# ZYM-PKU/UDiffText

Measured on AMD Instinct MI355X. Metric: 512x512 50-step denoised images/sec (UDiffText hot path: conditioner + 50 CFG Euler steps + VAE decode), higher is better.
Workload: dtype bf16; 1 GPU; 512x512, 50 Euler/DDIM(eta 0) steps, CFG 5.0, 9-char labels, noise_iters 0; global batch 4 per step sharded over 1 GPU(s) = 4 images per GPU in micro-batches of 4: every UNet call runs ONE batch of 4 (8 samples with CFG); 3 such batch(es) in flight per GPU on separate launch streams; BASELINE.json configs[1]; global_batch=4, weights=synthetic (name-keyed recipe), 1361.2 M parameters, launch=hipGraph replay of the sampler steps, in_flight=3, batches_per_unet_call=1

## Files before the change

### include/udt_kernels.h

```cpp
#ifndef UDT_KERNELS_H
#define UDT_KERNELS_H

#include <stddef.h>
#include <stdint.h>

#ifdef __cplusplus
extern "C" {
#endif

typedef enum {
  UDT_OK = 0,
  UDT_ERR_BAD_SHAPE = -1,
  UDT_ERR_BAD_ARG = -2,
  UDT_ERR_WORKSPACE = -3,
  UDT_ERR_HIP = -4,
  UDT_ERR_NO_DEVICE = -5,
  UDT_ERR_ASYNC = -6
} udt_status;

typedef enum {
  UDT_DTYPE_F32 = 0,
  UDT_DTYPE_BF16 = 1,
  UDT_DTYPE_FP8_E4M3 = 2
} udt_dtype;
// ... 94 lines not shown
                          int32_t batch, int32_t nq, int32_t nk,
                          int32_t ldq, int32_t ldk, int32_t ldv, int32_t ldo,
                          int64_t q_bstride, int64_t k_bstride, int64_t v_bstride, int64_t o_bstride,
                          float scale, void* workspace, size_t workspace_bytes, void* stream);

int udt_mattn_fwd(const void* q, const void* k, const void* v, void* o, const float* mask, const uint8_t* kpm,
                  int32_t batch, int32_t heads, int32_t head_dim, int32_t nq, int32_t lk,
                  int32_t ldq, int32_t ldk, int32_t ldv, int32_t ldo, int32_t ldmask,
                  int64_t q_bstride, int64_t k_bstride, int64_t v_bstride, int64_t o_bstride, float scale, void* stream);

int32_t udt_tattn_hp(int32_t heads);
int udt_tattn_prepare(const void* kv, int32_t ldkv, const void* wq, int32_t ldwq, const void* wo, int32_t ldwo,
                      const float* gamma, const float* beta, void* A, float* sc, void* BmT, int32_t B, int32_t L,
                      int32_t C, int32_t heads, float scale, void* stream);
int udt_tattn_fused(const void* x, void* out, const void* A, const float* sc, const void* BmT, const float* bias,
                    int32_t B, int32_t n_tok, int32_t C, int32_t heads, int32_t zero_samples, float eps, void* stream);
int32_t udt_tattn_rowstat_parts(int32_t B, int32_t n_tok, int32_t C);
int udt_tattn_fused_q8(const void* x, void* out, const void* A, const float* sc, const void* BmT, const float* bias,
                       int32_t B, int32_t n_tok, int32_t C, int32_t heads, int32_t zero_samples, float eps, void* q8_out,
                       void* q8_scale, float* rowstat_out, void* stream);

int udt_softmax_rows(void* x, int64_t rows, int32_t cols, int32_t ld, void* stream);

int32_t udt_gn_nchunks(int64_t HW, int32_t C);
int udt_gn_stats(const void* x, const void* x2, float* partials, int32_t B, int64_t HW, int32_t C, int32_t C2,
                 int32_t G, void* stream);
int udt_gn_apply(const void* x, const void* x2, void* y, const float* partials, const float* gamma,
                 const float* beta, int32_t B, int64_t HW, int32_t C, int32_t C2, int32_t G, float eps, int32_t act,
                 void* stream);
int32_t udt_gn_strip_ok(int32_t B, int64_t HW, int32_t C1, int32_t C2, int32_t G);
int udt_gn_strip(const void* x, const void* x2, void* y, const float* gamma, const float* beta, int32_t B, int64_t HW,
// ... 175 lines not shown
```

### udifftext_amd/csrc/common.h

```cpp
#pragma once
#include <hip/hip_runtime.h>
#include <stdint.h>
#include "../../include/udt_kernels.h"

typedef __attribute__((ext_vector_type(8))) __bf16 bf16x8_t;
typedef __attribute__((ext_vector_type(2))) __bf16 bf16x2_t;
typedef __attribute__((ext_vector_type(2))) float f32x2;
typedef __attribute__((ext_vector_type(4))) float f32x4;
typedef __attribute__((ext_vector_type(16))) float f32x16;
typedef __attribute__((ext_vector_type(2))) uint32_t u32x2;
typedef __attribute__((ext_vector_type(4))) uint32_t u32x4;

#define UDT_DEVINL __device__ __forceinline__

#ifdef UDT_MEASURE
#define UDT_DBG(flags, bit) ((((flags) >> (bit)) & 1) != 0)
#else
#define UDT_DBG(flags, bit) false
#endif

UDT_DEVINL float bf16_bits_to_f32(uint32_t v) { return __uint_as_float(v << 16); }
UDT_DEVINL float bf16_lo(uint32_t packed) { return __uint_as_float(packed << 16); }
UDT_DEVINL float bf16_hi(uint32_t packed) { return __uint_as_float(packed & 0xffff0000u); }

// ... 162 lines not shown
UDT_DEVINL float xor32_sum(float v) {
  const auto r = __builtin_amdgcn_permlane32_swap(__builtin_bit_cast(unsigned, v), __builtin_bit_cast(unsigned, v), false, false);
  return __builtin_bit_cast(float, (unsigned)r[0]) + __builtin_bit_cast(float, (unsigned)r[1]);
}

int udt_set_hip_error(hipError_t e);
const uint16_t* udt_zero_page();

struct UdtProfScope {
  int cls; hipStream_t s; void* rec;
  UdtProfScope(int cls_, hipStream_t s_);
  ~UdtProfScope();
};

void udt_prof_tag(void* rec, const char* tag);

#define UDT_CHECK_LAUNCH()                                   \
  do {                                                       \
    hipError_t _e = hipGetLastError();                       \
    if (_e != hipSuccess) return udt_set_hip_error(_e);      \
  } while (0)
```

### udifftext_amd/csrc/gemm.hip

```cpp
#include "common.h"
#include <stdio.h>
#include <stdlib.h>
#include <string.h>
#include <atomic>
#include <cmath>

hipError_t udt_lean_launch_gemm(int cfg, const void* lparams, int smem, int G, int geglu, int ln, hipStream_t s);
hipError_t udt_lean_launch_conv3(const void* c3params, hipStream_t s);

namespace {
#include "tile_common.h"

struct GemmParams {
  const uint16_t* a;
  const uint16_t* a2;
  const uint16_t* w;
  const uint16_t* zero;
  const float* bias;
  const uint16_t* res;
  const float* rowvec;
  void* out;
  const float* colscale;
  const float* in_scsh;
  float* colstats;
// ... 966 lines not shown
  if (lean_plan(d, lt, true)) {
    rows = lt.stats_rows;
    slots = lt.tiles_m * (lt.bm / lt.stats_rows);
    return true;
  }
  return false;
}
}

extern "C" int udt_debug_set(const char* key, int32_t value) {
  if (!key) return UDT_ERR_BAD_ARG;
  if (!strcmp(key, "n_block")) { g_n_block.store(value); return UDT_OK; }
  if (!strcmp(key, "rows_epi")) { g_rows_epi.store(value ? 1 : 0); return UDT_OK; }
  if (!strcmp(key, "lean")) { g_lean.store(value < 0 ? -2 : value); return UDT_OK; }
  if (!strcmp(key, "rowres")) { g_rowres.store(value < 0 ? 1 : (value ? 1 : 0)); return UDT_OK; }
  if (!strcmp(key, "wide_lanes_eff")) { g_wide_lanes_eff.store(value < 0 ? -2 : value); return UDT_OK; }
  if (!strcmp(key, "conv_n4")) { g_conv_n4.store(value < 0 ? -2 : (value ? 1 : 0)); return UDT_OK; }
  if (!strcmp(key, "lean256_lanes")) { g_lean256_lanes.store(value < 0 ? -2 : (value ? 1 : 0)); return UDT_OK; }
  if (!strcmp(key, "lean_splitk")) { g_lean_splitk.store(value); return UDT_OK; }
  if (!strcmp(key, "share_splitk")) { g_share_splitk.store(value < 0 ? -2 : (value ? 1 : 0)); return UDT_OK; }
  if (!strcmp(key, "lean_conv")) { g_lean_conv.store(value < 0 ? -1 : (value ? 1 : 0)); return UDT_OK; }
  if (!strcmp(key, "wide_conv")) { g_wide_conv.store(value < 0 ? -1 : (value ? 1 : 0)); return UDT_OK; }
#ifdef UDT_MEASURE
  if (!strcmp(key, "lconv_dbg")) { g_lconv_dbg.store(value); return UDT_OK; }
  static const struct { const char* k; int bit; } bits[] = {{"no_xchg", 28}, {"no_epi", 27}, {"no_store", 26}, {"no_res", 25},
                                                            {"no_bias", 24}, {"no_fast", 22}};
  for (const auto& b : bits)
    if (!strcmp(key, b.k)) {
      int cur = g_dbg_bits.load();
      g_dbg_bits.store((cur & ~(1 << b.bit)) | (value ? (1 << b.bit) : 0));
// ... 390 lines not shown
```

### udifftext_amd/csrc/tattn.hip

```cpp
#include "common.h"
#include <stdio.h>
#include <stdlib.h>

namespace {

constexpr int TA_THREADS = 512;
constexpr int TA_WAVES = TA_THREADS / 64;

struct TattnParams {
  const uint16_t* x;
  uint16_t* out;
  const uint16_t* A;
  const float* sc;
  const uint16_t* BmT;
  const float* bias;
  const uint16_t* zero;
  int M, C, hp, n_tok, zero_samples;
  int nsplit;
  float eps;
  uint8_t* q8_out;
  uint32_t* q8_scale;
  float* rowstat_out;
};

UDT_DEVINL f32x16 zero16() {
  f32x16 z;
#pragma unroll
  for (int r = 0; r < 16; ++r) z[r] = 0.f;
  return z;
}

template <int TT, int NKT, int NKS, bool Q8 = false>
__global__ void __launch_bounds__(TA_THREADS) tattn_fused_kernel(const TattnParams p) {
  extern __shared__ __attribute__((aligned(16))) char smem[];
  constexpr int C = NKT * 64, hp = NKS * 16;
  constexpr int nkt = NKT;
  constexpr int TA_AHEAD = NKT <= 10 ? NKT : 8;
  char* const xs = smem;
  float* const stats = reinterpret_cast<float*>(smem + (size_t)nkt * TT * 128);
  const int prs = hp * 2 + 16;
  char* const pl = reinterpret_cast<char*>(stats + TT * 2);
  const int tid = threadIdx.x;
  const int wave = __builtin_amdgcn_readfirstlane(tid >> 6);
  const int lane = tid & 63;
  const int l31 = lane & 31, hi = lane >> 5;
  const long long tok0 = (long long)blockIdx.x * TT;
  const int b = (int)(tok0 / p.n_tok);
  const uint16_t* xg = p.x + tok0 * C;
  uint16_t* og = p.out + tok0 * C;
  float* const rst = reinterpret_cast<float*>(pl + (size_t)TT * prs);
  const int ct_lo = (int)blockIdx.y * (C >> 5) / p.nsplit, ct_hi = ((int)blockIdx.y + 1) * (C >> 5) / p.nsplit;
  auto q8_row_stats = [&]() {
    __syncthreads();
    if (tid < TT && tok0 + tid < p.M) {
      float s = 0.f, q = 0.f;
      for (int ct = ct_lo; ct < ct_hi; ++ct) {
        const f32x2 v = *reinterpret_cast<const f32x2*>(rst + ((size_t)tid * (C >> 5) + ct) * 2);
        s += v[0];
        q += v[1];
      }
      f32x2 o = {s, q};
      reinterpret_cast<f32x2*>(p.rowstat_out)[(long long)blockIdx.y * p.M + tok0 + tid] = o;
    }
  };


  const uint16_t* Ab = p.A + (long long)b * hp * C;
  constexpr int jt = hp >> 5;
  constexpr int tiles1 = jt * (TT / 32);
// ... 2 lines not shown
  if (live && wave < tiles1) {
    const uint16_t* arow = Ab + (long long)(wave / (TT / 32)) * (32 * C) + lane * 8;
#pragma unroll
    for (int u = 0; u < TA_AHEAD; ++u)
#pragma unroll
      for (int ks = 0; ks < 4; ++ks) ar[u][ks] = *reinterpret_cast<const bf16x8_t*>(arow + (u * 4 + ks) * 512);
  }

  {
    const int pieces = nkt * (TT / 8);
    const int l3 = lane >> 3, ps = lane & 7;
    for (int pc = wave; pc < pieces; pc += TA_WAVES) {
      const int kt = pc / (TT / 8), rg = pc - kt * (TT / 8);
      const int row = rg * 8 + l3;
      const int slot = ps ^ ((row >> 1) & 7);
      const uint16_t* src = (tok0 + row < p.M) ? (xg + (long long)row * C + kt * 64 + slot * 8) : p.zero;
      glds16(src, xs + (size_t)pc * 1024);
    }
    wait_vmcnt0();
  }
  __syncthreads();

  if (b < p.zero_samples) {
    const int ch_lo = ct_lo * 4, ch_hi = ct_hi * 4;
    const int nch = ch_hi - ch_lo;
    for (int i0 = 0; i0 < TT * nch; i0 += TA_THREADS) {
      const int i = i0 + tid;
      const bool act = i < TT * nch;
      const int row = act ? i / nch : 0, ch = ch_lo + (act ? i - row * nch : 0);
      const bool ok = act && tok0 + row < p.M;
      const int kt = ch >> 3, s = ch & 7;
      const u32x4 v = *reinterpret_cast<const u32x4*>(xs + ((size_t)kt * TT + row) * 128 + ((s ^ ((row >> 1) & 7)) << 4));
      const f32x4 b0 = *reinterpret_cast<const f32x4*>(p.bias + ch * 8), b1 = *reinterpret_cast<const f32x4*>(p.bias + ch * 8 + 4);
      const float f[8] = {bf16_lo(v[0]) + b0[0], bf16_hi(v[0]) + b0[1], bf16_lo(v[1]) + b0[2], bf16_hi(v[1]) + b0[3],
                          bf16_lo(v[2]) + b1[0], bf16_hi(v[2]) + b1[1], bf16_lo(v[3]) + b1[2], bf16_hi(v[3]) + b1[3]};
      u32x4 o = {pack_bf16x2(f[0], f[1]), pack_bf16x2(f[2], f[3]), pack_bf16x2(f[4], f[5]), pack_bf16x2(f[6], f[7])};
      if (ok) *reinterpret_cast<u32x4*>(og + (long long)row * C + ch * 8) = o;
      if constexpr (Q8) {
        uint32_t sb;
        const u32x2 q8 = mx8_quant_row8(f, sb);
        float ps = 0.f, pq = 0.f;
#pragma unroll
        for (int j = 0; j < 8; ++j) ps += f[j], pq += f[j] * f[j];
        ps = dpp_add<0xB1>(ps); pq = dpp_add<0xB1>(pq);
        ps = dpp_add<0x4E>(ps); pq = dpp_add<0x4E>(pq);
// ... 61 lines not shown
      bf16x8_t af[4], xf[4];
#pragma unroll
      for (int ks = 0; ks < 4; ++ks) {
        af[ks] = ar[u][ks];
        xf[ks] = lds_read_frag(xrow + (((ks * 2 + hi) ^ swz) << 4));
      }
      if (kt + TA_AHEAD < nkt) {
#pragma unroll
        for (int ks = 0; ks < 4; ++ks) ar[u][ks] = *reinterpret_cast<const bf16x8_t*>(arow + ((kt + TA_AHEAD) * 4 + ks) * 512);
      }
#pragma unroll
      for (int ks = 0; ks < 4; ++ks) acc = mfma32(af[ks], xf[ks], acc);
    }
    const float mean = stats[row * 2], rstd = stats[row * 2 + 1];
    float sv[16];
#pragma unroll
    for (int r4 = 0; r4 < 4; ++r4) {
      const int j = ct * 32 + 8 * r4 + 4 * hi;
      const f32x4 c0 = *reinterpret_cast<const f32x4*>(scb + j * 2), c1 = *reinterpret_cast<const f32x4*>(scb + j * 2 + 4);
      sv[r4 * 4 + 0] = rstd * (acc[r4 * 4 + 0] - mean * c0[0]) + c0[1];
      sv[r4 * 4 + 1] = rstd * (acc[r4 * 4 + 1] - mean * c0[2]) + c0[3];
      sv[r4 * 4 + 2] = rstd * (acc[r4 * 4 + 2] - mean * c1[0]) + c1[1];
      sv[r4 * 4 + 3] = rstd * (acc[r4 * 4 + 3] - mean * c1[2]) + c1[3];
    }
#pragma unroll
    for (int h2 = 0; h2 < 2; ++h2) {
      float mx = sv[h2 * 8];
#pragma unroll
      for (int r = 1; r < 8; ++r) mx = fmaxf(mx, sv[h2 * 8 + r]);
      mx = fmaxf(mx, __shfl_xor(mx, 32));
      float sum = 0.f;
#pragma unroll
      for (int r = 0; r < 8; ++r) {
        sv[h2 * 8 + r] = __expf(sv[h2 * 8 + r] - mx);
        sum += sv[h2 * 8 + r];
      }
      sum += __shfl_xor(sum, 32);
      const float inv = 1.0f / sum;
#pragma unroll
      for (int r = 0; r < 8; ++r) sv[h2 * 8 + r] *= inv;
    }
#pragma unroll
    for (int r4 = 0; r4 < 4; ++r4) {
      const int j = ct * 32 + 8 * r4 + 4 * hi;
      u32x2 pk = {pack_bf16x2(sv[r4 * 4], sv[r4 * 4 + 1]), pack_bf16x2(sv[r4 * 4 + 2], sv[r4 * 4 + 3])};
      *reinterpret_cast<u32x2*>(pl + (size_t)row * prs + j * 2) = pk;
    }
  }
  __syncthreads();

  const uint16_t* Bb = p.BmT + (long long)b * C * hp;
  const int tiles2 = (ct_hi - ct_lo) * (TT / 32);
  constexpr int nks = NKS;
  for (int t = wave; t < tiles2; t += TA_WAVES) {
    const int rt = t % (TT / 32), ct = ct_lo + t / (TT / 32);
    const int row = rt * 32 + l31;
    const uint16_t* brow = Bb + (long long)ct * (32 * hp) + lane * 8;
    const char* prow = pl + (size_t)row * prs + hi * 16;
    f32x16 acc = zero16();
    bf16x8_t bn[NKS];
#pragma unroll
    for (int i = 0; i < NKS; ++i) bn[i] = *reinterpret_cast<const bf16x8_t*>(brow + i * 512);
#pragma unroll
    for (int ks = 0; ks < nks; ++ks) {
      const bf16x8_t pf = *reinterpret_cast<const bf16x8_t*>(prow + ks * 32);
      acc = mfma32(bn[ks], pf, acc);
    }
    {
      const bool rok = tok0 + row < p.M;
      const int swz = (row >> 1) & 7;
      float v[16];
#pragma unroll
      for (int r4 = 0; r4 < 4; ++r4) {
        const int c = ct * 32 + 8 * r4 + 4 * hi;
        const f32x4 bv = *reinterpret_cast<const f32x4*>(p.bias + c);
        const int kt = c >> 6, sl = (c & 63) >> 3;
        const u32x2 xr = *reinterpret_cast<const u32x2*>(xs + ((size_t)kt * TT + row) * 128 + ((sl ^ swz) << 4) + (c & 7) * 2);
        v[r4 * 4 + 0] = acc[r4 * 4 + 0] + bv[0] + bf16_lo(xr[0]);
        v[r4 * 4 + 1] = acc[r4 * 4 + 1] + bv[1] + bf16_hi(xr[0]);
        v[r4 * 4 + 2] = acc[r4 * 4 + 2] + bv[2] + bf16_lo(xr[1]);
        v[r4 * 4 + 3] = acc[r4 * 4 + 3] + bv[3] + bf16_hi(xr[1]);
        u32x2 pk = {pack_bf16x2(v[r4 * 4 + 0], v[r4 * 4 + 1]), pack_bf16x2(v[r4 * 4 + 2], v[r4 * 4 + 3])};
        if (rok) *reinterpret_cast<u32x2*>(og + (long long)row * C + c) = pk;
      }
// ... 7 lines not shown
        pq = xor32_sum(pq);
        if (rok) {
          const long long m = tok0 + row;
#pragma unroll
          for (int r4 = 0; r4 < 4; ++r4) *reinterpret_cast<uint32_t*>(p.q8_out + m * C + ct * 32 + 8 * r4 + 4 * hi) = q[r4];
          if (hi == 0) {
            reinterpret_cast<uint8_t*>(p.q8_scale)[((long long)(ct >> 2) * p.M + m) * 4 + (ct & 3)] = (uint8_t)sb;
            f32x2 st2 = {ps, pq};
            *reinterpret_cast<f32x2*>(rst + ((size_t)row * (C >> 5) + ct) * 2) = st2;
          }
        }
      }
    }
  }
  if constexpr (Q8) q8_row_stats();
}

__global__ void __launch_bounds__(256) tattn_prepare_a_kernel(const uint16_t* __restrict__ kv, int ldkv, const uint16_t* __restrict__ wq,
                                                              int ldwq, const float* __restrict__ gamma, const float* __restrict__ beta,
                                                              uint16_t* __restrict__ A, float* __restrict__ sc, int L, int C, int hp,
                                                              int heads, float scale) {
  __shared__ float kvec[64];
  __shared__ float red[2][4];
  const int j = blockIdx.x, b = blockIdx.y, t = threadIdx.x;
  const int h = j >> 4, i = j & 15;
  uint16_t* const Ab = A + (long long)b * hp * C;
  const int nkt = C >> 6;
  auto aoff = [&](int k) {
    return ((((long long)(j >> 5) * nkt + (k >> 6)) * 4 + ((k >> 4) & 3)) * 64 + ((k >> 3) & 1) * 32 + (j & 31)) * 8 + (k & 7);
  };
// ... 58 lines not shown
  hipStream_t s = reinterpret_cast<hipStream_t>(stream);
  UdtProfScope prof(3, s);
  hipLaunchKernelGGL(tattn_prepare_a_kernel, dim3(hp, B), dim3(256), 0, s, reinterpret_cast<const uint16_t*>(kv), ldkv,
                     reinterpret_cast<const uint16_t*>(wq), ldwq, gamma, beta, reinterpret_cast<uint16_t*>(A), sc, L, C, hp, heads, scale);
  UDT_CHECK_LAUNCH();
  const long long n = (long long)B * C * hp;
  hipLaunchKernelGGL(tattn_prepare_b_kernel, dim3((unsigned)((n + 255) / 256)), dim3(256), 0, s,
                     reinterpret_cast<const uint16_t*>(kv), ldkv, C, reinterpret_cast<const uint16_t*>(wo), ldwo,
                     reinterpret_cast<uint16_t*>(BmT), B, L, C, hp, heads);
  UDT_CHECK_LAUNCH();
  return UDT_OK;
}

namespace {
int tattn_tt(int C) { return C >= 640 ? 32 : 64; }
int tattn_nsplit(int M, int TT) {
  const unsigned grid = (unsigned)(M / TT);
  constexpr unsigned target = 256u;
  int nsplit = 1;
  while (nsplit < 8 && grid * nsplit < target) nsplit *= 2;
  return nsplit;
}

int tattn_launch(const void* x, void* out, const void* A, const float* sc, const void* BmT, const float* bias, int32_t B, int32_t n_tok,
                 int32_t C, int32_t heads, int32_t zero_samples, float eps, void* q8_out, void* q8_scale, float* rowstat_out, void* stream) {
  if (!x || !out || !bias || (zero_samples < B && (!A || !sc || !BmT))) return UDT_ERR_BAD_ARG;
  if (B <= 0 || n_tok <= 0 || heads <= 0 || C != heads * 64 || C > 1280 || zero_samples < 0 || zero_samples > B) return UDT_ERR_BAD_SHAPE;
  const int TT = tattn_tt(C);
  if (n_tok % TT != 0) return UDT_ERR_BAD_SHAPE;
  const bool q8 = q8_out != nullptr;
  if (q8 && (!q8_scale || !rowstat_out || C % 128 != 0)) return UDT_ERR_BAD_ARG;
  TattnParams p;
  p.x = reinterpret_cast<const uint16_t*>(x); p.out = reinterpret_cast<uint16_t*>(out);
  p.A = reinterpret_cast<const uint16_t*>(A); p.sc = sc; p.BmT = reinterpret_cast<const uint16_t*>(BmT); p.bias = bias;
  p.zero = udt_zero_page();
  if (!p.zero) return UDT_ERR_HIP;
  p.M = B * n_tok; p.C = C; p.hp = udt_tattn_hp(heads); p.n_tok = n_tok; p.zero_samples = zero_samples; p.eps = eps;
  p.q8_out = reinterpret_cast<uint8_t*>(q8_out); p.q8_scale = reinterpret_cast<uint32_t*>(q8_scale); p.rowstat_out = rowstat_out;
  const size_t smem = (size_t)TT * C * 2 + (size_t)TT * 2 * sizeof(float) + (size_t)TT * (p.hp * 2 + 16) + (q8 ? (size_t)TT * (C / 32) * 8 : 0);
  hipStream_t s = reinterpret_cast<hipStream_t>(stream);
  UdtProfScope prof(3, s);
  if (prof.rec) {
    char tag[96];
    snprintf(tag, sizeof(tag), "tattn_fused%s B=%d n=%d C=%d zero=%d", q8 ? "+q8" : "", B, n_tok, C, zero_samples);
    udt_prof_tag(prof.rec, tag);
  }
  static bool attr_done[5] = {false, false, false, false, false};
  const unsigned grid = (unsigned)(p.M / TT);
  p.nsplit = tattn_nsplit(p.M, TT);
  const void* fn = nullptr;
  int which = -1;
  if (C == 320 && p.hp == 96 && !q8) { fn = reinterpret_cast<const void*>(tattn_fused_kernel<64, 5, 6>); which = 0; }
  else if (C == 640 && p.hp == 160) { fn = q8 ? reinterpret_cast<const void*>(tattn_fused_kernel<32, 10, 10, true>) : reinterpret_cast<const void*>(tattn_fused_kernel<32, 10, 10>); which = q8 ? 3 : 1; }
  else if (C == 1280 && p.hp == 320) { fn = q8 ? reinterpret_cast<const void*>(tattn_fused_kernel<32, 20, 20, true>) : reinterpret_cast<const void*>(tattn_fused_kernel<32, 20, 20>); which = q8 ? 4 : 2; }
  else return UDT_ERR_BAD_SHAPE;
  if (!attr_done[which]) {
    hipError_t e = hipFuncSetAttribute(fn, hipFuncAttributeMaxDynamicSharedMemorySize, 128 * 1024);
    if (e != hipSuccess) return udt_set_hip_error(e);
    attr_done[which] = true;
  }
  void* args[] = {&p};
  hipError_t el = hipLaunchKernel(fn, dim3(grid, p.nsplit), dim3(TA_THREADS), args, smem, s);
  if (el != hipSuccess) return udt_set_hip_error(el);
  UDT_CHECK_LAUNCH();
  return UDT_OK;
}
}

extern "C" int udt_tattn_fused(const void* x, void* out, const void* A, const float* sc, const void* BmT, const float* bias,
                               int32_t B, int32_t n_tok, int32_t C, int32_t heads, int32_t zero_samples, float eps, void* stream) {
  return tattn_launch(x, out, A, sc, BmT, bias, B, n_tok, C, heads, zero_samples, eps, nullptr, nullptr, nullptr, stream);
}

extern "C" int32_t udt_tattn_rowstat_parts(int32_t B, int32_t n_tok, int32_t C) {
  if (B <= 0 || n_tok <= 0 || (C != 640 && C != 1280)) return 0;
  const int TT = tattn_tt(C);
  if (n_tok % TT != 0) return 0;
  return tattn_nsplit(B * n_tok, TT);
}

extern "C" int udt_tattn_fused_q8(const void* x, void* out, const void* A, const float* sc, const void* BmT, const float* bias,
                                  int32_t B, int32_t n_tok, int32_t C, int32_t heads, int32_t zero_samples, float eps, void* q8_out,
                                  void* q8_scale, float* rowstat_out, void* stream) {
  if (!q8_out) return UDT_ERR_BAD_ARG;
  return tattn_launch(x, out, A, sc, BmT, bias, B, n_tok, C, heads, zero_samples, eps, q8_out, q8_scale, rowstat_out, stream);
}
```

### udifftext_amd/lib.py

```python
from __future__ import annotations

import ctypes as C
import os

_HERE = os.path.dirname(os.path.abspath(__file__))
LIB_PATH = os.path.join(_HERE, "libudt_kernels.so")

GEMM_OUT_F32 = 1 << 0
DTYPE_F32, DTYPE_BF16, DTYPE_FP8_E4M3 = 0, 1, 2
GEMM_GEGLU = 1 << 1
GEMM_RELU = 1 << 2
GEMM_TRANSPOSED = 1 << 3
GEMM_CONV = 1 << 4
GEMM_SILU_OUT = 1 << 5
GEMM_MX8 = 1 << 7

PROF_CONV3X3, PROF_GEMM, PROF_ATTN, PROF_XATTN, PROF_NORM, PROF_ELEMENTWISE = range(6)


class GemmDesc(C.Structure):
    _fields_ = [
        ("a", C.c_void_p), ("a2", C.c_void_p), ("w", C.c_void_p), ("bias", C.c_void_p),
        ("residual", C.c_void_p), ("rowvec", C.c_void_p), ("out", C.c_void_p),
        ("M", C.c_int32), ("N", C.c_int32), ("K", C.c_int32),
# ... 63 lines not shown
    "udt_attn_rowv_fwd": (C.c_int, [_vp, _vp, _vp, _vp, _i32, _i32, _i32, _i32, _i32, _i32, _i32, _i32,
                                    _i64, _i64, _i64, _i64, _f32, _vp]),
    "udt_attn_rowv_q8_fwd": (C.c_int, [_vp, _vp, _vp, _vp, _i32, _i32, _i32, _i32, _i32, _i32, _i32, _i32,
                                       _i64, _i64, _i64, _i64, _f32, _vp, _vp, _i32, _vp]),
    "udt_attn_mx8_fwd": (C.c_int, [_vp, _vp, _vp, _i32, _i32, _i32, _i32, _i32, _f32, _f32, _vp, _vp, _i32, _vp]),
    "udt_attn512_fwd": (C.c_int, [_vp, _vp, _vp, _vp, _i32, _i32, _i32, _i32, _i32, _i32, _i32, _i64, _i64, _i64, _i64, _f32, _vp]),
    "udt_attn512_workspace_bytes": (C.c_size_t, [_i32, _i32, _i32]),
    "udt_attn512_split_fwd": (C.c_int, [_vp, _vp, _vp, _vp, _i32, _i32, _i32, _i32, _i32, _i32, _i32, _i64, _i64, _i64, _i64, _f32,
                                        _vp, C.c_size_t, _vp]),
    "udt_xattn_fwd": (C.c_int, [_vp, _vp, _vp, _vp, _fp, _i32, _i32, _i32, _i32, _i32, _i32, _i32, _i32, _f32, _vp]),
    "udt_mattn_fwd": (C.c_int, [_vp, _vp, _vp, _vp, _fp, _vp, _i32, _i32, _i32, _i32, _i32, _i32, _i32, _i32, _i32, _i32,
                                _i64, _i64, _i64, _i64, _f32, _vp]),
    "udt_softmax_rows": (C.c_int, [_vp, _i64, _i32, _i32, _vp]),
    "udt_tattn_hp": (_i32, [_i32]),
    "udt_tattn_prepare": (C.c_int, [_vp, _i32, _vp, _i32, _vp, _i32, _fp, _fp, _vp, _fp, _vp, _i32, _i32, _i32, _i32, _f32, _vp]),
    "udt_tattn_fused": (C.c_int, [_vp, _vp, _vp, _fp, _vp, _fp, _i32, _i32, _i32, _i32, _i32, _f32, _vp]),
    "udt_tattn_rowstat_parts": (_i32, [_i32, _i32, _i32]),
    "udt_tattn_fused_q8": (C.c_int, [_vp, _vp, _vp, _fp, _vp, _fp, _i32, _i32, _i32, _i32, _i32, _f32, _vp, _vp, _fp, _vp]),
    "udt_gn_nchunks": (_i32, [_i64, _i32]),
    "udt_gn_stats": (C.c_int, [_vp, _vp, _fp, _i32, _i64, _i32, _i32, _i32, _vp]),
    "udt_gn_apply": (C.c_int, [_vp, _vp, _vp, _fp, _fp, _fp, _i32, _i64, _i32, _i32, _i32, _f32, _i32, _vp]),
    "udt_gn_strip_ok": (_i32, [_i32, _i64, _i32, _i32, _i32]),
    "udt_gn_strip": (C.c_int, [_vp, _vp, _vp, _fp, _fp, _i32, _i64, _i32, _i32, _i32, _f32, _i32, _vp]),
    "udt_layernorm": (C.c_int, [_vp, _vp, _fp, _fp, _i64, _i32, _f32, _vp]),
    "udt_unet_input": (C.c_int, [_fp, _vp, _i32, _i32, _i32, _f32, _vp]),
    "udt_unet_input_churn": (C.c_int, [_fp, _fp, _vp, _i32, _i32, _i32, _f32, _f32, _vp]),
    "udt_cfg_euler_step": (C.c_int, [_fp, _fp, _fp, _i32, _i32, _i32, _f32, _f32, _f32, _f32, _vp]),
    "udt_cfg_sampler_step": (C.c_int, [_fp, _fp, _fp, _fp, _fp, _fp, _fp, _i32, _i32, _i32, SamplerCoefs, _vp]),
    "udt_cfg_multistep_step": (C.c_int, [_fp, _fp, _fp, _fp, _i32, _i32, _i32, MultistepCoefs, _vp]),
    "udt_precond_unet_input": (C.c_int, [_fp, _fp, _vp, _i32, _i32, _i32, _f32, _f32, _i32, _vp]),
    "udt_precond_euler_step": (C.c_int, [_fp, _fp, _fp, _i32, _i32, _i32, _f32, _f32, _f32, _f32, _f32, _i32, _vp]),
# ... 96 lines not shown
```

### udifftext_amd/ops.py

```python
from __future__ import annotations

import contextlib
import ctypes as C
import os
import threading
from typing import NamedTuple, Optional, Sequence

import torch

from . import lib as L

WORKSPACE_BYTES = 96 << 20


class Workspace:

    def __init__(self, device, nbytes: int = WORKSPACE_BYTES):
        if torch.device(device).type != "cuda":
            raise L.UdtError("udifftext_amd workspaces live on the GPU (no CPU fallback)")
        self.buf = torch.zeros(nbytes, dtype=torch.uint8, device=device)

    def check(self, stream: Optional[int] = None) -> None:
        L.check(L.load().udt_check_async_error(self.buf.data_ptr(), self.buf.numel(), _stream() if stream is None else stream),
                "udt_check_async_error")


class _Ctx(threading.local):
# ... 530 lines not shown
        out = torch.empty_like(x)
    assert out.is_contiguous()
    if tables is not None:
        assert tables.A.is_contiguous() and tables.sc.is_contiguous() and tables.BmT.is_contiguous() and tables.A.shape[0] == B
    if getattr(out, "mx8", None) is not None:
        del out.mx8
    parts = L.load().udt_tattn_rowstat_parts(B, N, Cc) if emit_q8 else 0
    if parts > 0:
        q = _mx8_alloc(B * N, Cc, x.device)
        q = Mx8Act(q.data, q.scale, torch.empty((parts, B * N, 2), dtype=torch.float32, device=x.device))
        L.check(L.load().udt_tattn_fused_q8(_ptr(x), _ptr(out), _ptr(tables.A) if tables else None, _ptr(tables.sc) if tables else None,
                                            _ptr(tables.BmT) if tables else None, _ptr(bias), B, N, Cc, heads, zero_samples, eps,
                                            _ptr(q.data), _ptr(q.scale), _ptr(q.stats), _stream()), "udt_tattn_fused_q8")
        out.mx8 = q
        return out
    L.check(L.load().udt_tattn_fused(_ptr(x), _ptr(out), _ptr(tables.A) if tables else None, _ptr(tables.sc) if tables else None,
                                     _ptr(tables.BmT) if tables else None, _ptr(bias), B, N, Cc, heads, zero_samples, eps, _stream()),
            "udt_tattn_fused")
    return out


def softmax_rows_(x: torch.Tensor) -> torch.Tensor:
    _bf16(x)
    assert x.is_contiguous()
    cols = x.shape[-1]
    L.check(L.load().udt_softmax_rows(_ptr(x), x.numel() // cols, cols, cols, _stream()), "udt_softmax_rows")
    return x


def group_norm(x: torch.Tensor, gamma: torch.Tensor, beta: torch.Tensor, groups: int, eps: float, silu: bool,
               out: Optional[torch.Tensor] = None, x2: Optional[torch.Tensor] = None) -> torch.Tensor:
    _bf16(x)
    assert x.is_contiguous()
# ... 630 lines not shown
```

Before: 10.46 images/s.

## Split fused text-attention into scores and output kernels at C=1280

Adds a two-kernel path for the fused text cross-attention. The first kernel computes layernorm stats, QK scores and softmax, writing bf16 probabilities to workspace scratch. The second kernel computes the output projection, bias and residual, and its grid is split across channel slices. Work is ordered with an XCD-aware block mapping and pairs of zero and live samples. By default the path is enabled only for C=1280, where the fused kernel had few tiles and therefore low parallelism. The cost is an extra launch plus a round-trip of the probabilities through global memory.

```diff
diff --git a/include/udt_kernels.h b/include/udt_kernels.h
--- a/include/udt_kernels.h
+++ b/include/udt_kernels.h
@@ -132,7 +132,8 @@
                       const float* gamma, const float* beta, void* A, float* sc, void* BmT, int32_t B, int32_t L,
                       int32_t C, int32_t heads, float scale, void* stream);
 int udt_tattn_fused(const void* x, void* out, const void* A, const float* sc, const void* BmT, const float* bias,
-                    int32_t B, int32_t n_tok, int32_t C, int32_t heads, int32_t zero_samples, float eps, void* stream);
+                    int32_t B, int32_t n_tok, int32_t C, int32_t heads, int32_t zero_samples, float eps, void* scratch,
+                    size_t scratch_bytes, void* stream);
 int32_t udt_tattn_rowstat_parts(int32_t B, int32_t n_tok, int32_t C);
 int udt_tattn_fused_q8(const void* x, void* out, const void* A, const float* sc, const void* BmT, const float* bias,
                        int32_t B, int32_t n_tok, int32_t C, int32_t heads, int32_t zero_samples, float eps, void* q8_out,
diff --git a/udifftext_amd/csrc/common.h b/udifftext_amd/csrc/common.h
--- a/udifftext_amd/csrc/common.h
+++ b/udifftext_amd/csrc/common.h
@@ -200,6 +200,7 @@
 };
 
 void udt_prof_tag(void* rec, const char* tag);
+void udt_tattn_debug_split(int v);
 
 #define UDT_CHECK_LAUNCH()                                   \
   do {                                                       \
diff --git a/udifftext_amd/csrc/gemm.hip b/udifftext_amd/csrc/gemm.hip
--- a/udifftext_amd/csrc/gemm.hip
+++ b/udifftext_amd/csrc/gemm.hip
@@ -1004,6 +1004,7 @@
   if (!strcmp(key, "rows_epi")) { g_rows_epi.store(value ? 1 : 0); return UDT_OK; }
   if (!strcmp(key, "lean")) { g_lean.store(value < 0 ? -2 : value); return UDT_OK; }
   if (!strcmp(key, "rowres")) { g_rowres.store(value < 0 ? 1 : (value ? 1 : 0)); return UDT_OK; }
+  if (!strcmp(key, "tattn_split")) { udt_tattn_debug_split(value); return UDT_OK; }
   if (!strcmp(key, "wide_lanes_eff")) { g_wide_lanes_eff.store(value < 0 ? -2 : value); return UDT_OK; }
   if (!strcmp(key, "conv_n4")) { g_conv_n4.store(value < 0 ? -2 : (value ? 1 : 0)); return UDT_OK; }
   if (!strcmp(key, "lean256_lanes")) { g_lean256_lanes.store(value < 0 ? -2 : (value ? 1 : 0)); return UDT_OK; }
diff --git a/udifftext_amd/csrc/tattn.hip b/udifftext_amd/csrc/tattn.hip
--- a/udifftext_amd/csrc/tattn.hip
+++ b/udifftext_amd/csrc/tattn.hip
@@ -1,6 +1,7 @@
 #include "common.h"
 #include <stdio.h>
 #include <stdlib.h>
+#include <atomic>
 
 namespace {
 
@@ -16,11 +17,14 @@
   const float* bias;
   const uint16_t* zero;
   int M, C, hp, n_tok, zero_samples;
+  int tps;
   int nsplit;
   float eps;
   uint8_t* q8_out;
   uint32_t* q8_scale;
   float* rowstat_out;
+  uint16_t* pscr;
+  int cpb, nblk;
 };
 
 UDT_DEVINL f32x16 zero16() {
@@ -28,6 +32,35 @@
 #pragma unroll
   for (int r = 0; r < 16; ++r) z[r] = 0.f;
   return z;
+}
+
+UDT_DEVINL void tattn_softmax_tile(const f32x16& acc, float mean, float rstd, const float* scb, int ct, int hi, float (&sv)[16]) {
+#pragma unroll
+  for (int r4 = 0; r4 < 4; ++r4) {
+    const int j = ct * 32 + 8 * r4 + 4 * hi;
+    const f32x4 c0 = *reinterpret_cast<const f32x4*>(scb + j * 2), c1 = *reinterpret_cast<const f32x4*>(scb + j * 2 + 4);
+    sv[r4 * 4 + 0] = rstd * (acc[r4 * 4 + 0] - mean * c0[0]) + c0[1];
+    sv[r4 * 4 + 1] = rstd * (acc[r4 * 4 + 1] - mean * c0[2]) + c0[3];
+    sv[r4 * 4 + 2] = rstd * (acc[r4 * 4 + 2] - mean * c1[0]) + c1[1];
+    sv[r4 * 4 + 3] = rstd * (acc[r4 * 4 + 3] - mean * c1[2]) + c1[3];
+  }
+#pragma unroll
+  for (int h2 = 0; h2 < 2; ++h2) {
+    float mx = sv[h2 * 8];
+#pragma unroll
+    for (int r = 1; r < 8; ++r) mx = fmaxf(mx, sv[h2 * 8 + r]);
+    mx = fmaxf(mx, __shfl_xor(mx, 32));
+    float sum = 0.f;
+#pragma unroll
+    for (int r = 0; r < 8; ++r) {
+      sv[h2 * 8 + r] = __expf(sv[h2 * 8 + r] - mx);
+      sum += sv[h2 * 8 + r];
+    }
+    sum += __shfl_xor(sum, 32);
+    const float inv = 1.0f / sum;
+#pragma unroll
+    for (int r = 0; r < 8; ++r) sv[h2 * 8 + r] *= inv;
+  }
 }
 
 template <int TT, int NKT, int NKS, bool Q8 = false>
@@ -44,15 +77,16 @@
   const int wave = __builtin_amdgcn_readfirstlane(tid >> 6);
   const int lane = tid & 63;
   const int l31 = lane & 31, hi = lane >> 5;
-  const long long tok0 = (long long)blockIdx.x * TT;
-  const int b = (int)(tok0 / p.n_tok);
+  const int b = (int)blockIdx.x / p.tps, t0 = ((int)blockIdx.x - b * p.tps) * TT;
+  const long long tok0 = (long long)b * p.n_tok + t0;
+  const int nrow = min(TT, p.n_tok - t0);
   const uint16_t* xg = p.x + tok0 * C;
   uint16_t* og = p.out + tok0 * C;
   float* const rst = reinterpret_cast<float*>(pl + (size_t)TT * prs);
   const int ct_lo = (int)blockIdx.y * (C >> 5) / p.nsplit, ct_hi = ((int)blockIdx.y + 1) * (C >> 5) / p.nsplit;
   auto q8_row_stats = [&]() {
     __syncthreads();
-    if (tid < TT && tok0 + tid < p.M) {
+    if (tid < nrow) {
       float s = 0.f, q = 0.f;
       for (int ct = ct_lo; ct < ct_hi; ++ct) {
         const f32x2 v = *reinterpret_cast<const f32x2*>(rst + ((size_t)tid * (C >> 5) + ct) * 2);
@@ -85,7 +119,7 @@
       const int kt = pc / (TT / 8), rg = pc - kt * (TT / 8);
       const int row = rg * 8 + l3;
       const int slot = ps ^ ((row >> 1) & 7);
-      const uint16_t* src = (tok0 + row < p.M) ? (xg + (long long)row * C + kt * 64 + slot * 8) : p.zero;
+      const uint16_t* src = (row < nrow) ? (xg + (long long)row * C + kt * 64 + slot * 8) : p.zero;
       glds16(src, xs + (size_t)pc * 1024);
     }
     wait_vmcnt0();
@@ -99,7 +133,7 @@
       const int i = i0 + tid;
       const bool act = i < TT * nch;
       const int row = act ? i / nch : 0, ch = ch_lo + (act ? i - row * nch : 0);
-      const bool ok = act && tok0 + row < p.M;
+      const bool ok = act && row < nrow;
       const int kt = ch >> 3, s = ch & 7;
       const u32x4 v = *reinterpret_cast<const u32x4*>(xs + ((size_t)kt * TT + row) * 128 + ((s ^ ((row >> 1) & 7)) << 4));
       const f32x4 b0 = *reinterpret_cast<const f32x4*>(p.bias + ch * 8), b1 = *reinterpret_cast<const f32x4*>(p.bias + ch * 8 + 4);
@@ -191,32 +225,7 @@
     }
     const float mean = stats[row * 2], rstd = stats[row * 2 + 1];
     float sv[16];
-#pragma unroll
-    for (int r4 = 0; r4 < 4; ++r4) {
-      const int j = ct * 32 + 8 * r4 + 4 * hi;
-      const f32x4 c0 = *reinterpret_cast<const f32x4*>(scb + j * 2), c1 = *reinterpret_cast<const f32x4*>(scb + j * 2 + 4);
-      sv[r4 * 4 + 0] = rstd * (acc[r4 * 4 + 0] - mean * c0[0]) + c0[1];
-      sv[r4 * 4 + 1] = rstd * (acc[r4 * 4 + 1] - mean * c0[2]) + c0[3];
-      sv[r4 * 4 + 2] = rstd * (acc[r4 * 4 + 2] - mean * c1[0]) + c1[1];
-      sv[r4 * 4 + 3] = rstd * (acc[r4 * 4 + 3] - mean * c1[2]) + c1[3];
-    }
-#pragma unroll
-    for (int h2 = 0; h2 < 2; ++h2) {
-      float mx = sv[h2 * 8];
-#pragma unroll
-      for (int r = 1; r < 8; ++r) mx = fmaxf(mx, sv[h2 * 8 + r]);
-      mx = fmaxf(mx, __shfl_xor(mx, 32));
-      float sum = 0.f;
-#pragma unroll
-      for (int r = 0; r < 8; ++r) {
-        sv[h2 * 8 + r] = __expf(sv[h2 * 8 + r] - mx);
-        sum += sv[h2 * 8 + r];
-      }
-      sum += __shfl_xor(sum, 32);
-      const float inv = 1.0f / sum;
-#pragma unroll
-      for (int r = 0; r < 8; ++r) sv[h2 * 8 + r] *= inv;
-    }
+    tattn_softmax_tile(acc, mean, rstd, scb, ct, hi, sv);
 #pragma unroll
     for (int r4 = 0; r4 < 4; ++r4) {
       const int j = ct * 32 + 8 * r4 + 4 * hi;
@@ -244,7 +253,7 @@
       acc = mfma32(bn[ks], pf, acc);
     }
     {
-      const bool rok = tok0 + row < p.M;
+      const bool rok = row < nrow;
       const int swz = (row >> 1) & 7;
       float v[16];
 #pragma unroll
@@ -282,6 +291,196 @@
     }
   }
   if constexpr (Q8) q8_row_stats();
+}
+
+UDT_DEVINL int tattn_xcd_chunk(int bid, int nwg) {
+  const int q = nwg >> 3, r = nwg & 7, x = bid & 7;
+  return (x < r ? x * (q + 1) : r * (q + 1) + (x - r) * q) + (bid >> 3);
+}
+
+template <int NKT, int NKS>
+__global__ void __launch_bounds__(TA_THREADS) tattn_scores_kernel(const TattnParams p) {
+  extern __shared__ __attribute__((aligned(16))) char smem[];
+  constexpr int TT = 32, C = NKT * 64, hp = NKS * 16, nkt = NKT;
+  constexpr int TA_AHEAD = NKT <= 10 ? NKT : 8;
+  constexpr int jt = hp >> 5;
+  char* const xs = smem;
+  float* const stats = reinterpret_cast<float*>(smem + (size_t)nkt * TT * 128);
+  const int tid = threadIdx.x;
+  const int wave = __builtin_amdgcn_readfirstlane(tid >> 6);
+  const int lane = tid & 63;
+  const int l31 = lane & 31, hi = lane >> 5;
+  const int wg = tattn_xcd_chunk((int)blockIdx.x, (int)gridDim.x);
+  const int tile = wg / p.nblk + p.zero_samples * p.tps;
+  const int b = tile / p.tps, t0 = (tile - b * p.tps) * TT;
+  const long long tok0 = (long long)b * p.n_tok + t0;
+  const int nrow = min(TT, p.n_tok - t0);
+  const uint16_t* xg = p.x + tok0 * C;
+  const int ct = (wg % p.nblk) * p.cpb + wave;
+  const bool mine = wave < p.cpb && ct < jt;
+
+  const uint16_t* arow = p.A + (long long)b * hp * C + (long long)ct * (32 * C) + lane * 8;
+  bf16x8_t ar[TA_AHEAD][4];
+  if (mine) {
+#pragma unroll
+    for (int u = 0; u < TA_AHEAD; ++u)
+#pragma unroll
+      for (int ks = 0; ks < 4; ++ks) ar[u][ks] = *reinterpret_cast<const bf16x8_t*>(arow + (u * 4 + ks) * 512);
+  }
+  {
+    const int pieces = nkt * (TT / 8);
+    const int l3 = lane >> 3, ps = lane & 7;
+    for (int pc = wave; pc < pieces; pc += TA_WAVES) {
+      const int kt = pc / (TT / 8), rg = pc - kt * (TT / 8);
+      const int row = rg * 8 + l3;
+      const int slot = ps ^ ((row >> 1) & 7);
+      const uint16_t* src = (row < nrow) ? (xg + (long long)row * C + kt * 64 + slot * 8) : p.zero;
+      glds16(src, xs + (size_t)pc * 1024);
+    }
+    wait_vmcnt0();
+  }
+  __syncthreads();
+  {
+    constexpr int TPR = TA_THREADS / TT;
+    const int row = tid / TPR, part = tid - row * TPR;
+    const int swz = (row >> 1) & 7;
+    float s = 0.f, q = 0.f;
+    for (int ch = part; ch < nkt * 8; ch += TPR) {
+      const int kt = ch >> 3, sl = ch & 7;
+      const u32x4 v = *reinterpret_cast<const u32x4*>(xs + ((size_t)kt * TT + row) * 128 + ((sl ^ swz) << 4));
+#pragma unroll
+      for (int j = 0; j < 4; ++j) {
+        const float a = bf16_lo(v[j]), bb = bf16_hi(v[j]);
+        s += a + bb;
+        q += a * a + bb * bb;
+      }
+    }
+    s = dpp_add<0xB1>(s); q = dpp_add<0xB1>(q);
+    s = dpp_add<0x4E>(s); q = dpp_add<0x4E>(q);
+    s += __shfl_xor(s, 4); q += __shfl_xor(q, 4);
+    s += __shfl_xor(s, 8); q += __shfl_xor(q, 8);
+    if (part == 0) {
+      const float mean = s / (float)C;
+      float var = q / (float)C - mean * mean;
+      if (var < 0.f) var = 0.f;
+      stats[row * 2] = mean;
+      stats[row * 2 + 1] = rsqrtf(var + p.eps);
+    }
+  }
+  __syncthreads();
+  if (!mine) return;
+
+  const int row = l31;
+  const int swz = (l31 >> 1) & 7;
+  f32x16 acc = zero16();
+#pragma unroll
+  for (int kt = 0; kt < nkt; ++kt) {
+    const int u = kt % TA_AHEAD;
+    const char* xrow = xs + ((size_t)kt * TT + row) * 128;
+    bf16x8_t af[4], xf[4];
+#pragma unroll
+    for (int ks = 0; ks < 4; ++ks) {
+      af[ks] = ar[u][ks];
+      xf[ks] = lds_read_frag(xrow + (((ks * 2 + hi) ^ swz) << 4));
+    }
+    if (kt + TA_AHEAD < nkt) {
+#pragma unroll
+      for (int ks = 0; ks < 4; ++ks) ar[u][ks] = *reinterpret_cast<const bf16x8_t*>(arow + ((kt + TA_AHEAD) * 4 + ks) * 512);
+    }
+#pragma unroll
+    for (int ks = 0; ks < 4; ++ks) acc = mfma32(af[ks], xf[ks], acc);
+  }
+  float sv[16];
+  tattn_softmax_tile(acc, stats[row * 2], stats[row * 2 + 1], p.sc + (long long)b * hp * 2, ct, hi, sv);
+  uint16_t* const pg = p.pscr + ((long long)tile * TT + row) * hp;
+#pragma unroll
+  for (int r4 = 0; r4 < 4; ++r4) {
+    const int j = ct * 32 + 8 * r4 + 4 * hi;
+    u32x2 pk = {pack_bf16x2(sv[r4 * 4], sv[r4 * 4 + 1]), pack_bf16x2(sv[r4 * 4 + 2], sv[r4 * 4 + 3])};
+    *reinterpret_cast<u32x2*>(pg + j) = pk;
+  }
+}
+
+template <int NKT, int NKS>
+__global__ void __launch_bounds__(TA_THREADS) tattn_out_kernel(const TattnParams p) {
+  constexpr int TT = 32, C = NKT * 64, hp = NKS * 16;
+  const int tid = threadIdx.x;
+  const int wave = __builtin_amdgcn_readfirstlane(tid >> 6);
+  const int lane = tid & 63;
+  const int l31 = lane & 31, hi = lane >> 5;
+  const int wg = tattn_xcd_chunk((int)blockIdx.x, (int)gridDim.x);
+  const int u = wg / p.nsplit, split = wg - u * p.nsplit;
+  int b, t;
+  {
+    const int Z = p.zero_samples, Bn = p.M / p.n_tok;
+    const int m = min(Z, Bn - Z);
+    if (u < 2 * m * p.tps) {
+      const int pr = u / (2 * p.tps), w = u - pr * 2 * p.tps;
+      b = (w & 1) ? Z + pr : pr;
+      t = w >> 1;
+    } else {
+      const int ur = u - 2 * m * p.tps, rs = ur / p.tps;
+      b = rs < Z - m ? m + rs : Z + m + (rs - (Z - m));
+      t = ur - rs * p.tps;
+    }
+  }
+  const int tile = b * p.tps + t, t0 = t * TT;
+  const long long tok0 = (long long)b * p.n_tok + t0;
+  const int nrow = min(TT, p.n_tok - t0);
+  const uint16_t* xg = p.x + tok0 * C;
+  uint16_t* og = p.out + tok0 * C;
+  const int ct_lo = split * (C >> 5) / p.nsplit, ct_hi = (split + 1) * (C >> 5) / p.nsplit;
+
+  if (b < p.zero_samples) {
+    const int ch_lo = ct_lo * 4, nch = (ct_hi - ct_lo) * 4;
+    for (int i = tid; i < TT * nch; i += TA_THREADS) {
+      const int row = i / nch, ch = ch_lo + (i - row * nch);
+      if (row >= nrow) continue;
+      const u32x4 v = *reinterpret_cast<const u32x4*>(xg + (long long)row * C + ch * 8);
+      const f32x4 b0 = *reinterpret_cast<const f32x4*>(p.bias + ch * 8), b1 = *reinterpret_cast<const f32x4*>(p.bias + ch * 8 + 4);
+      const float f[8] = {bf16_lo(v[0]) + b0[0], bf16_hi(v[0]) + b0[1], bf16_lo(v[1]) + b0[2], bf16_hi(v[1]) + b0[3],
+                          bf16_lo(v[2]) + b1[0], bf16_hi(v[2]) + b1[1], bf16_lo(v[3]) + b1[2], bf16_hi(v[3]) + b1[3]};
+      u32x4 o = {pack_bf16x2(f[0], f[1]), pack_bf16x2(f[2], f[3]), pack_bf16x2(f[4], f[5]), pack_bf16x2(f[6], f[7])};
+      *reinterpret_cast<u32x4*>(og + (long long)row * C + ch * 8) = o;
+    }
+    return;
+  }
+
+  const int row = l31;
+  const bool rok = row < nrow;
+  if (wave >= ct_hi - ct_lo) return;
+  const uint16_t* prow = p.pscr + ((long long)tile * TT + row) * hp + hi * 8;
+  bf16x8_t pf[NKS];
+#pragma unroll
+  for (int ks = 0; ks < NKS; ++ks) pf[ks] = *reinterpret_cast<const bf16x8_t*>(prow + ks * 16);
+  const uint16_t* Bb = p.BmT + (long long)b * C * hp;
+  for (int ct = ct_lo + wave; ct < ct_hi; ct += TA_WAVES) {
+    const uint16_t* brow = Bb + (long long)ct * (32 * hp) + lane * 8;
+    bf16x8_t bn[NKS];
+#pragma unroll
+    for (int i = 0; i < NKS; ++i) bn[i] = *reinterpret_cast<const bf16x8_t*>(brow + i * 512);
+    u32x2 xr[4];
+#pragma unroll
+    for (int r4 = 0; r4 < 4; ++r4) {
+      const int c = ct * 32 + 8 * r4 + 4 * hi;
+      u32x2 z = {0u, 0u};
+      xr[r4] = rok ? *reinterpret_cast<const u32x2*>(xg + (long long)row * C + c) : z;
+    }
+    f32x16 acc = zero16();
+#pragma unroll
+    for (int ks = 0; ks < NKS; ++ks) acc = mfma32(bn[ks], pf[ks], acc);
+#pragma unroll
+    for (int r4 = 0; r4 < 4; ++r4) {
+      const int c = ct * 32 + 8 * r4 + 4 * hi;
+      const f32x4 bv = *reinterpret_cast<const f32x4*>(p.bias + c);
+      const float v0 = acc[r4 * 4 + 0] + bv[0] + bf16_lo(xr[r4][0]);
+      const float v1 = acc[r4 * 4 + 1] + bv[1] + bf16_hi(xr[r4][0]);
+      const float v2 = acc[r4 * 4 + 2] + bv[2] + bf16_lo(xr[r4][1]);
+      const float v3 = acc[r4 * 4 + 3] + bv[3] + bf16_hi(xr[r4][1]);
+      u32x2 pk = {pack_bf16x2(v0, v1), pack_bf16x2(v2, v3)};
+      if (rok) *reinterpret_cast<u32x2*>(og + (long long)row * C + c) = pk;
+    }
+  }
 }
 
 __global__ void __launch_bounds__(256) tattn_prepare_a_kernel(const uint16_t* __restrict__ kv, int ldkv, const uint16_t* __restrict__ wq,
@@ -370,74 +569,134 @@
 
 namespace {
 int tattn_tt(int C) { return C >= 640 ? 32 : 64; }
-int tattn_nsplit(int M, int TT) {
-  const unsigned grid = (unsigned)(M / TT);
+int tattn_nsplit(int tiles) {
   constexpr unsigned target = 256u;
   int nsplit = 1;
-  while (nsplit < 8 && grid * nsplit < target) nsplit *= 2;
+  while (nsplit < 8 && (unsigned)tiles * nsplit < target) nsplit *= 2;
   return nsplit;
 }
 
+std::atomic<int> g_tattn_split{-1};
+
+constexpr int TATTN_SCORE_TILES_PER_WG = 2;
+
+bool tattn_split_auto(int C) { return C == 1280; }
+
+struct TattnPlan {
+  int TT, tps, tiles, nsplit;
+  bool split;
+  size_t scratch;
+};
+TattnPlan tattn_plan(int B, int n_tok, int C, bool q8) {
+  TattnPlan pl;
+  pl.TT = tattn_tt(C);
+  pl.tps = (n_tok + pl.TT - 1) / pl.TT;
+  pl.tiles = B * pl.tps;
+  pl.nsplit = tattn_nsplit(pl.tiles);
+  const bool can = pl.nsplit > 1 && pl.TT == 32 && !q8;
+  const int mode = g_tattn_split.load(std::memory_order_relaxed);
+  pl.split = mode < 0 ? (can && tattn_split_auto(C)) : (mode > 0 && can);
+  pl.scratch = (size_t)pl.tiles * 32 * (size_t)udt_tattn_hp(C / 64) * 2;
+  return pl;
+}
+
 int tattn_launch(const void* x, void* out, const void* A, const float* sc, const void* BmT, const float* bias, int32_t B, int32_t n_tok,
-                 int32_t C, int32_t heads, int32_t zero_samples, float eps, void* q8_out, void* q8_scale, float* rowstat_out, void* stream) {
+                 int32_t C, int32_t heads, int32_t zero_samples, float eps, void* q8_out, void* q8_scale, float* rowstat_out,
+                 void* scratch, size_t scratch_bytes, void* stream) {
   if (!x || !out || !bias || (zero_samples < B && (!A || !sc || !BmT))) return UDT_ERR_BAD_ARG;
   if (B <= 0 || n_tok <= 0 || heads <= 0 || C != heads * 64 || C > 1280 || zero_samples < 0 || zero_samples > B) return UDT_ERR_BAD_SHAPE;
-  const int TT = tattn_tt(C);
-  if (n_tok % TT != 0) return UDT_ERR_BAD_SHAPE;
   const bool q8 = q8_out != nullptr;
   if (q8 && (!q8_scale || !rowstat_out || C % 128 != 0)) return UDT_ERR_BAD_ARG;
+  TattnPlan pl = tattn_plan(B, n_tok, C, q8);
+  const int TT = pl.TT;
+  if (q8 && n_tok % TT != 0) return UDT_ERR_BAD_SHAPE;
+  if ((long long)pl.tiles * TT > 0x7fffffffLL / 2) return UDT_ERR_BAD_SHAPE;
+  const int forced = g_tattn_split.load(std::memory_order_relaxed);
+  if (forced > 0 && pl.nsplit > 1 && !pl.split && !q8) return UDT_ERR_BAD_SHAPE;
+  if (pl.split && (!scratch || scratch_bytes < pl.scratch || (reinterpret_cast<uintptr_t>(scratch) & 15))) {
+    if (forced > 0) return UDT_ERR_BAD_ARG;
+    pl.split = false;
+  }
   TattnParams p;
   p.x = reinterpret_cast<const uint16_t*>(x); p.out = reinterpret_cast<uint16_t*>(out);
   p.A = reinterpret_cast<const uint16_t*>(A); p.sc = sc; p.BmT = reinterpret_cast<const uint16_t*>(BmT); p.bias = bias;
   p.zero = udt_zero_page();
   if (!p.zero) return UDT_ERR_HIP;
   p.M = B * n_tok; p.C = C; p.hp = udt_tattn_hp(heads); p.n_tok = n_tok; p.zero_samples = zero_samples; p.eps = eps;
+  p.tps = pl.tps; p.nsplit = pl.nsplit;
   p.q8_out = reinterpret_cast<uint8_t*>(q8_out); p.q8_scale = reinterpret_cast<uint32_t*>(q8_scale); p.rowstat_out = rowstat_out;
-  const size_t smem = (size_t)TT * C * 2 + (size_t)TT * 2 * sizeof(float) + (size_t)TT * (p.hp * 2 + 16) + (q8 ? (size_t)TT * (C / 32) * 8 : 0);
+  p.pscr = reinterpret_cast<uint16_t*>(scratch); p.cpb = TATTN_SCORE_TILES_PER_WG;
+  p.nblk = ((p.hp >> 5) + p.cpb - 1) / p.cpb;
   hipStream_t s = reinterpret_cast<hipStream_t>(stream);
   UdtProfScope prof(3, s);
   if (prof.rec) {
     char tag[96];
-    snprintf(tag, sizeof(tag), "tattn_fused%s B=%d n=%d C=%d zero=%d", q8 ? "+q8" : "", B, n_tok, C, zero_samples);
+    snprintf(tag, sizeof(tag), "tattn_fused%s B=%d n=%d C=%d zero=%d%s", q8 ? "+q8" : "", B, n_tok, C, zero_samples, pl.split ? " two-kernel" : "");
     udt_prof_tag(prof.rec, tag);
   }
-  static bool attr_done[5] = {false, false, false, false, false};
-  const unsigned grid = (unsigned)(p.M / TT);
-  p.nsplit = tattn_nsplit(p.M, TT);
+  static bool attr_done[7] = {false, false, false, false, false, false, false};
+  auto max_lds = [&](const void* fn, int which) {
+    if (attr_done[which]) return hipSuccess;
+    hipError_t e = hipFuncSetAttribute(fn, hipFuncAttributeMaxDynamicSharedMemorySize, 128 * 1024);
+    if (e == hipSuccess) attr_done[which] = true;
+    return e;
+  };
+  void* args[] = {&p};
+  if (pl.split) {
+    const void *fs = nullptr, *fo = nullptr;
+    int which = -1;
+    if (C == 640 && p.hp == 160) { fs = reinterpret_cast<const void*>(tattn_scores_kernel<10, 10>); fo = reinterpret_cast<const void*>(tattn_out_kernel<10, 10>); which = 5; }
+    else if (C == 1280 && p.hp == 320) { fs = reinterpret_cast<const void*>(tattn_scores_kernel<20, 20>); fo = reinterpret_cast<const void*>(tattn_out_kernel<20, 20>); which = 6; }
+    else return UDT_ERR_BAD_SHAPE;
+    const int live = (B - zero_samples) * pl.tps;
+    if (live > 0) {
+      hipError_t e = max_lds(fs, which);
+      if (e != hipSuccess) return udt_set_hip_error(e);
+      const size_t smem_s = (size_t)TT * C * 2 + (size_t)TT * 2 * sizeof(float);
+      e = hipLaunchKernel(fs, dim3((unsigned)(live * p.nblk)), dim3(TA_THREADS), args, smem_s, s);
+      if (e != hipSuccess) return udt_set_hip_error(e);
+      UDT_CHECK_LAUNCH();
+    }
+    hipError_t e = hipLaunchKernel(fo, dim3((unsigned)(pl.tiles * pl.nsplit)), dim3(TA_THREADS), args, 0, s);
+    if (e != hipSuccess) return udt_set_hip_error(e);
+    UDT_CHECK_LAUNCH();
+    return UDT_OK;
+  }
+  const size_t smem = (size_t)TT * C * 2 + (size_t)TT * 2 * sizeof(float) + (size_t)TT * (p.hp * 2 + 16) + (q8 ? (size_t)TT * (C / 32) * 8 : 0);
   const void* fn = nullptr;
   int which = -1;
   if (C == 320 && p.hp == 96 && !q8) { fn = reinterpret_cast<const void*>(tattn_fused_kernel<64, 5, 6>); which = 0; }
   else if (C == 640 && p.hp == 160) { fn = q8 ? reinterpret_cast<const void*>(tattn_fused_kernel<32, 10, 10, true>) : reinterpret_cast<const void*>(tattn_fused_kernel<32, 10, 10>); which = q8 ? 3 : 1; }
   else if (C == 1280 && p.hp == 320) { fn = q8 ? reinterpret_cast<const void*>(tattn_fused_kernel<32, 20, 20, true>) : reinterpret_cast<const void*>(tattn_fused_kernel<32, 20, 20>); which = q8 ? 4 : 2; }
   else return UDT_ERR_BAD_SHAPE;
-  if (!attr_done[which]) {
-    hipError_t e = hipFuncSetAttribute(fn, hipFuncAttributeMaxDynamicSharedMemorySize, 128 * 1024);
-    if (e != hipSuccess) return udt_set_hip_error(e);
-    attr_done[which] = true;
-  }
-  void* args[] = {&p};
-  hipError_t el = hipLaunchKernel(fn, dim3(grid, p.nsplit), dim3(TA_THREADS), args, smem, s);
+  hipError_t e = max_lds(fn, which);
+  if (e != hipSuccess) return udt_set_hip_error(e);
+  hipError_t el = hipLaunchKernel(fn, dim3((unsigned)pl.tiles, p.nsplit), dim3(TA_THREADS), args, smem, s);
   if (el != hipSuccess) return udt_set_hip_error(el);
   UDT_CHECK_LAUNCH();
   return UDT_OK;
 }
 }
 
+void udt_tattn_debug_split(int v) { g_tattn_split.store(v < 0 ? -1 : (v ? 1 : 0)); }
+
 extern "C" int udt_tattn_fused(const void* x, void* out, const void* A, const float* sc, const void* BmT, const float* bias,
-                               int32_t B, int32_t n_tok, int32_t C, int32_t heads, int32_t zero_samples, float eps, void* stream) {
-  return tattn_launch(x, out, A, sc, BmT, bias, B, n_tok, C, heads, zero_samples, eps, nullptr, nullptr, nullptr, stream);
+                               int32_t B, int32_t n_tok, int32_t C, int32_t heads, int32_t zero_samples, float eps, void* scratch,
+                               size_t scratch_bytes, void* stream) {
+  return tattn_launch(x, out, A, sc, BmT, bias, B, n_tok, C, heads, zero_samples, eps, nullptr, nullptr, nullptr, scratch, scratch_bytes,
+                      stream);
 }
 
 extern "C" int32_t udt_tattn_rowstat_parts(int32_t B, int32_t n_tok, int32_t C) {
   if (B <= 0 || n_tok <= 0 || (C != 640 && C != 1280)) return 0;
   const int TT = tattn_tt(C);
   if (n_tok % TT != 0) return 0;
-  return tattn_nsplit(B * n_tok, TT);
+  return tattn_nsplit(B * n_tok / TT);
 }
 
 extern "C" int udt_tattn_fused_q8(const void* x, void* out, const void* A, const float* sc, const void* BmT, const float* bias,
                                   int32_t B, int32_t n_tok, int32_t C, int32_t heads, int32_t zero_samples, float eps, void* q8_out,
                                   void* q8_scale, float* rowstat_out, void* stream) {
   if (!q8_out) return UDT_ERR_BAD_ARG;
-  return tattn_launch(x, out, A, sc, BmT, bias, B, n_tok, C, heads, zero_samples, eps, q8_out, q8_scale, rowstat_out, stream);
-}
+  return tattn_launch(x, out, A, sc, BmT, bias, B, n_tok, C, heads, zero_samples, eps, q8_out, q8_scale, rowstat_out, nullptr, 0, stream);
+}
diff --git a/udifftext_amd/lib.py b/udifftext_amd/lib.py
--- a/udifftext_amd/lib.py
+++ b/udifftext_amd/lib.py
@@ -101,7 +101,7 @@
     "udt_softmax_rows": (C.c_int, [_vp, _i64, _i32, _i32, _vp]),
     "udt_tattn_hp": (_i32, [_i32]),
     "udt_tattn_prepare": (C.c_int, [_vp, _i32, _vp, _i32, _vp, _i32, _fp, _fp, _vp, _fp, _vp, _i32, _i32, _i32, _i32, _f32, _vp]),
-    "udt_tattn_fused": (C.c_int, [_vp, _vp, _vp, _fp, _vp, _fp, _i32, _i32, _i32, _i32, _i32, _f32, _vp]),
+    "udt_tattn_fused": (C.c_int, [_vp, _vp, _vp, _fp, _vp, _fp, _i32, _i32, _i32, _i32, _i32, _f32, _vp, C.c_size_t, _vp]),
     "udt_tattn_rowstat_parts": (_i32, [_i32, _i32, _i32]),
     "udt_tattn_fused_q8": (C.c_int, [_vp, _vp, _vp, _fp, _vp, _fp, _i32, _i32, _i32, _i32, _i32, _f32, _vp, _vp, _fp, _vp]),
     "udt_gn_nchunks": (_i32, [_i64, _i32]),
diff --git a/udifftext_amd/ops.py b/udifftext_amd/ops.py
--- a/udifftext_amd/ops.py
+++ b/udifftext_amd/ops.py
@@ -11,6 +11,7 @@
 from . import lib as L
 
 WORKSPACE_BYTES = 96 << 20
+WS_HEADER_BYTES = 4096
 
 
 class Workspace:
@@ -571,9 +572,13 @@
                                             _ptr(q.data), _ptr(q.scale), _ptr(q.stats), _stream()), "udt_tattn_fused_q8")
         out.mx8 = q
         return out
+    scr, scr_bytes = None, 0
+    if Cc >= 640 and not (_ctx.workspace is None and torch.cuda.is_current_stream_capturing()):
+        ws = _ws(WS_HEADER_BYTES, x.device)
+        scr, scr_bytes = ws.data_ptr() + WS_HEADER_BYTES, ws.numel() - WS_HEADER_BYTES
     L.check(L.load().udt_tattn_fused(_ptr(x), _ptr(out), _ptr(tables.A) if tables else None, _ptr(tables.sc) if tables else None,
-                                     _ptr(tables.BmT) if tables else None, _ptr(bias), B, N, Cc, heads, zero_samples, eps, _stream()),
-            "udt_tattn_fused")
+                                     _ptr(tables.BmT) if tables else None, _ptr(bias), B, N, Cc, heads, zero_samples, eps,
+                                     scr, scr_bytes, _stream()), "udt_tattn_fused")
     return out
 
 
```

New measurement: 10.50 images/s (median of 6 runs). No clear change (+0.4%).
